# IML-DKFZ/values

Measured on AMD Instinct MI355X. Metric: uncertainty-volumes/sec (64^3, T=10 MC-dropout), higher is better.
Workload: dtype f32; 1 GPU; C2: 64^3 1-channel volumes, UNet3D(initial_filter_size=8, 2 classes), T=10 MC-dropout passes + fused softmax/entropy/MI/variance/argmax reduction; dropout=hash bit generator, new seed every step, weights=torch default init, seed 123

## Files before the change

### values_amd/csrc/conv3d_deep.hip

```cpp
#include "s16_common.h"
#include "conv3d_internal.h"

struct DeepArgs {
  vx_conv3d_args a;
  const float* w;
  int tx, ty, tz, ts;
  int ltx, lty, ltz;
  int tiles_x, tiles_y, tiles_z;
  int npos;
  int nchunks, ncg;
  int npairs;
  unsigned m_cg, m_tx, m_ty, m_tz;
  int stat_epc;
  unsigned long long* stamps;
  int abl;
};

#define DP_STAMP VX_STAMP
#define DP_WAIT_LOADS VX_STAMP_WAIT_LOADS
#define DP_ABL VX_DIAG(ka.abl)

constexpr int DEEP_PREC_B = DEEP_NPOS * 16;
constexpr int DEEP_IMG_B = 2 * DEEP_PREC_B;

template <int R, int EPI, int PRE>
__global__ __launch_bounds__(768) void conv3d_deep_kernel(DeepArgs ka) {
  constexpr int NW = 8, NPW = 4, NTH = (NW + NPW) * 64, NST = NPW * 64;
  constexpr int NT = 2, NSTEP = 7;
  constexpr int IN_IT = R == 4 ? 9 : 7;
  constexpr int W_IT = DEEP_W_B / 16 / NST;
  constexpr bool STATS = EPI == 0;

  extern __shared__ __attribute__((aligned(16))) unsigned char smem_raw[];
  unsigned char* s_img = smem_raw;
  unsigned char* s_w = smem_raw + 2 * DEEP_IMG_B;
  float* s_red = reinterpret_cast<float*>(s_w + 2 * DEEP_W_B);
  float* s_bias = s_red + 2 * NW * 32 * 2;

  const vx_conv3d_args& a = ka.a;
  auto kernarg = [&]() {
    typedef const DeepArgs __attribute__((address_space(4))) * kp_t;
    kp_t p = (kp_t)__builtin_amdgcn_kernarg_segment_ptr();
    asm volatile("" : "+s"(p));
    return p;
  };
  const int tid = threadIdx.x, lane = tid & 63;
  const int wave = __builtin_amdgcn_readfirstlane(tid >> 6);
  const int m = lane & 15, g = lane >> 4;
  const int TX = ka.tx, TY = ka.ty, TZ = ka.tz;
  const int HX = TX + 2, HY = TY + 2, HZ = TZ + 2;
  const int NCH = ka.nchunks;

  for (int i = tid; i < a.Cout; i += NTH) s_bias[i] = a.bias[i];

  int vb = blockIdx.x;
  const int G = (int)gridDim.x;
  if ((G & 7) == 0) vb = (blockIdx.x & 7) * (G >> 3) + (blockIdx.x >> 3);
  const int npair_wg = vb < ka.npairs ? (ka.npairs - vb + G - 1) / G : 0;

  struct Cur { int ci, c; };
  auto advance = [&](Cur& x) { if (++x.c == NCH) { x.c = 0; ++x.ci; } };
  auto pair_of = [&](int ci, int& n0, int& tzi, int& tyi, int& txi, int& cg) {
    unsigned t = (unsigned)(vb + ci * G), q;
    q = ka.ncg == 1 ? t : __umulhi(t, ka.m_cg); cg = (int)(t - q * (unsigned)ka.ncg); t = q;
    q = ka.tiles_x == 1 ? t : __umulhi(t, ka.m_tx); txi = (int)(t - q * (unsigned)ka.tiles_x); t = q;
    q = ka.tiles_y == 1 ? t : __umulhi(t, ka.m_ty); tyi = (int)(t - q * (unsigned)ka.tiles_y); t = q;
    q = ka.tiles_z == 1 ? t : __umulhi(t, ka.m_tz); tzi = (int)(t - q * (unsigned)ka.tiles_z);
    n0 = (int)q * ka.ts;
  };

  float rmax = 0.f;
#ifdef VX_CONV_STAMPS
  unsigned long long st_sum[8] = {0, 0, 0, 0, 0, 0, 0, 0}, st_last, st_iters = 0;
  asm volatile("s_memtime %0\n\ts_waitcnt lgkmcnt(0)" : "=s"(st_last)::"memory");
#endif

  if (wave >= NW) {
    if constexpr (PRE != 0 || R == 2) __builtin_amdgcn_s_setprio(2);
    const int t = tid - NW * 64;
    const int q = t & 1;
    const int xb = a.in_xblk;
    const int Csrc = xb ? a.Cin / 2 : a.Cin;
    const int voxf = xb ? 2 * Csrc : a.in_pitch;
    const int rowf = a.W * voxf;
    const int biasf = (a.H + 1) * rowf + 4 * voxf;
    const size_t in_sample = (size_t)a.D * a.H * rowf;
    const int cper = xb ? Csrc / 8 : 0;
    const int lastx = (ka.tiles_x - 1) * TX, lasty = (ka.tiles_y - 1) * TY, lastz = (ka.tiles_z - 1) * TZ;
    unsigned voff[IN_IT];
    int ldst[IN_IT];
    unsigned ibad_always = 0, ibad_xlo = 0, ibad_xhi = 0, ibad_ylo = 0, ibad_yhi = 0, ibad_zlo = 0, ibad_zhi = 0;
    unsigned ibad_sge[3] = {0, 0, 0};
#pragma unroll
    for (int it = 0; it < IN_IT; ++it) {
      const int idx = t + it * NST;
      int vox = idx >> 1;
      if (vox >= ka.npos) { ibad_always |= 1u << it; vox = 0; }
      const int hx = vox % HX, r1 = vox / HX;
      const int hy = r1 % HY, r2 = r1 / HY;
      const int hz = r2 % HZ, smp = r2 / HZ;
      const int dxr = hx - 1, dyr = hy - 1, dzr = hz - 1;
      int xf;
      if (xb) {
        const int blk = dxr >= 0 ? dxr / xb : -((-dxr + xb - 1) / xb);
        const int rem = dxr - blk * xb;
        xf = (blk * 2) * xb * Csrc + rem * Csrc + 4 * q;
      } else {
        xf = dxr * a.in_pitch + 4 * q;
      }
      voff[it] = (unsigned)(((size_t)smp * in_sample + (size_t)((dzr * a.H + dyr) * rowf + xf + biasf)) * 4);
      ldst[it] = vox * 16 + q * 8;
      if (dxr < 0) ibad_xlo |= 1u << it;
      if (dxr >= a.W - lastx) ibad_xhi |= 1u << it;
      if (dyr < 0) ibad_ylo |= 1u << it;
      if (dyr >= a.H - lasty) ibad_yhi |= 1u << it;
      if (dzr < 0) ibad_zlo |= 1u << it;
      if (dzr >= a.D - lastz) ibad_zhi |= 1u << it;
#pragma unroll
      for (int k = 0; k < 3; ++k)
        if (smp > k) ibad_sge[k] |= 1u << it;
    }
    const uint32_t seed_in = PRE == 1 ? vx_seed_of(a, a.in_drop_seed) : 0u;

    f32x4 ibuf[IN_IT];
    f32x4 p_mean = {0.f, 0.f, 0.f, 0.f}, p_rstd = {1.f, 1.f, 1.f, 1.f};
    unsigned p_bad = 0xFFFFFFFFu, p_e0 = 0;
    vx_dkey p_key = {0u, 0u};
    unsigned cs_bad = 0xFFFFFFFFu, cs_soff = 0;
    int cs_n = 0;
    __amdgpu_buffer_rsrc_t cs_srd = __builtin_amdgcn_make_buffer_rsrc((void*)a.in, 0, 0, 0x00020000);
    auto pair_state = [&](int ci) {
      const bool have = ci < npair_wg;
      int n0 = 0, tzi = 0, tyi = 0, txi = 0, cg = 0;
      if (have) pair_of(ci, n0, tzi, tyi, txi, cg);
      unsigned bad = ibad_always;
      if (txi == 0) bad |= ibad_xlo;
      if (txi == ka.tiles_x - 1) bad |= ibad_xhi;
      if (tyi == 0) bad |= ibad_ylo;
      if (tyi == ka.tiles_y - 1) bad |= ibad_yhi;
      if (tzi == 0) bad |= ibad_zlo;
      if (tzi == ka.tiles_z - 1) bad |= ibad_zhi;
      const int nv = a.N - n0;
      if (nv < ka.ts) bad |= ibad_sge[nv >= 1 ? nv - 1 : 0];
      if (!have) bad = 0xFFFFFFFFu;
      cs_bad = bad;
      cs_soff = (unsigned)((((tzi * TZ) * a.H + tyi * TY) * rowf + txi * TX * voxf) * 4);
// ... 201 lines not shown
        for (int nt = 0; nt < NT; ++nt)
#pragma unroll
          for (int j = 0; j < 4; ++j) { ssum[nt][j] = 0.f; ssq[nt][j] = 0.f; }
      }
      int m_ = m;
      asm volatile("" : "+v"(m_));
#pragma unroll
      for (int r = 0; r < R; ++r) {
        int cx_, ly, lz, smp;
        vox_of((wave * R + r) * 16 + m_, cx_, ly, lz, smp);
        const int ovox = (lz * a.H + ly) * a.W + cx_;
        unsigned ovoff_r = ((unsigned)smp * (unsigned)out_sample + (unsigned)ovox * (unsigned)out_voxf + (unsigned)kp->a.out_coff + 4u * g) * 4u;
        if constexpr (R == 2) {
          if (n0 + smp >= a.N) ovoff_r = VX_OOB;
        }
        uint32_t hword = 0;
        if (EPI == 1) {
          const vx_dkey key = vx_drop_key(seed_out, kp->a.drop_layer, (uint32_t)(n0 + smp));
          hword = vx_drop_word(key, (vox0 + (unsigned)ovox) * (unsigned)ka.ncg + (unsigned)cg) >> (4 * g);
        }
#pragma unroll
        for (int nt = 0; nt < NT; ++nt) {
          f32x4 v;
#pragma unroll
          for (int j = 0; j < 4; ++j) v[j] = fmaf(accx[r][nt][j], 1.0f / 2048.f, acc[r][nt][j]);
          if (STATS) {
#pragma unroll
            for (int j = 0; j < 4; ++j) { ssum[nt][j] += v[j]; ssq[nt][j] = fmaf(v[j], v[j], ssq[nt][j]); }
          }
          if (f_lrelu) {
#pragma unroll
            for (int j = 0; j < 4; ++j) v[j] = fmaxf(v[j], 0.01f * v[j]);
          } else if (f_relu) {
#pragma unroll
            for (int j = 0; j < 4; ++j) v[j] = fmaxf(v[j], 0.f);
          }
          if (EPI == 1) {
            const uint32_t bits = hword >> (16 * nt);
#pragma unroll
            for (int j = 0; j < 4; ++j) v[j] *= __uint_as_float((bits << (30 - j)) & 0x40000000u);
          }
          if (!STATS) rmax = vx_max3abs(vx_max3abs(rmax, v[0], v[1]), v[2], v[3]);
          u32x4 sv = __builtin_bit_cast(u32x4, v);
          if (EPI == 1 || EPI == 3) {
            if (a.out_split) {
              typedef unsigned u32x2 __attribute__((ext_vector_type(2)));
              f16x4 hi, lo;
              vx_split4_s(v, hi, lo);
              const u32x2 h2 = __builtin_bit_cast(u32x2, hi), l2 = __builtin_bit_cast(u32x2, lo);
              sv = (u32x4){h2[0], h2[1], l2[0], l2[1]};
            }
          }
          __builtin_amdgcn_raw_buffer_store_b128(sv, osrd, (int)ovoff_r, (int)(osoff + (unsigned)(nt * 64)), 0);
          __builtin_amdgcn_sched_barrier(0);
          asm volatile("s_nop 3" ::: "memory");
          __builtin_amdgcn_sched_barrier(0);
        }
      }
      if (STATS) {
#pragma unroll
        for (int nt = 0; nt < NT; ++nt)
#pragma unroll
          for (int j = 0; j < 4; ++j) {
            float s = ssum[nt][j], qq = ssq[nt][j];
#pragma unroll
            for (int rot = 8; rot >= 1; rot >>= 1) { s += vx_row_ror(s, rot); qq += vx_row_ror(qq, rot); }
            if (m == 0) {
              red[(wave * 32 + nt * 16 + g * 4 + j) * 2 + 0] = s;
              red[(wave * 32 + nt * 16 + g * 4 + j) * 2 + 1] = qq;
            }
          }
      }
    };

    auto flush_tile = [&](int ci) {
      const float* red = s_red + (ci & 1) * (NW * 32 * 2);
      int n0, tzi, tyi, txi, cg;
      pair_of(ci, n0, tzi, tyi, txi, cg);
      const auto kp = kernarg();
      const int epc = kp->stat_epc;
      const int tps = ka.tiles_x * ka.tiles_y * ka.tiles_z;
      const int tile = (tzi * ka.tiles_y + tyi) * ka.tiles_x + txi;
      float* dst = kp->a.stats_partial + (((size_t)n0 * tps + tile) * epc * a.Cout + cg * 32) * 2;
      if (tid < 32) {
        float s = 0.f, qq = 0.f;
#pragma unroll
        for (int w = 0; w < NW; ++w) {
          s += red[(w * 32 + tid) * 2 + 0];
          qq += red[(w * 32 + tid) * 2 + 1];
        }
        dst[tid * 2 + 0] = s;
        dst[tid * 2 + 1] = qq;
      }
      for (int e = 1; e < epc; ++e)
        if (tid < 64) dst[(size_t)e * a.Cout * 2 + tid] = 0.f;
    };

    const bool late = wave >= NW / 2;
    Cur cx = {0, 0};
    int j = 0;
    int prev_ci = -1;
    int fl_ci = -1, fl_at = 0;
    while (cx.ci < npair_wg) {
      __syncthreads();
      DP_STAMP(0);
      if (STATS && fl_ci >= 0 && j >= fl_at && !late) { flush_tile(fl_ci); fl_ci = -1; }
      if (late && prev_ci >= 0) {
        if (!(DP_ABL & 2)) epilogue(prev_ci);
        prev_ci = -1;
      }
      DP_STAMP(2);
      if (cx.c == 0) {
        int n0, tzi, tyi, txi, cg;
        pair_of(cx.ci, n0, tzi, tyi, txi, cg);
        const f32x4 zero = {0.f, 0.f, 0.f, 0.f};
#pragma unroll
        for (int nt = 0; nt < NT; ++nt) {
          const f32x4 b4 = *reinterpret_cast<const f32x4*>(s_bias + cg * 32 + nt * 16 + 4 * g);
#pragma unroll
          for (int r = 0; r < R; ++r) { acc[r][nt] = b4; accx[r][nt] = zero; }
        }
      }
      if (!(DP_ABL & 1)) multiply(j & 1);
      DP_STAMP(1);
      if (cx.c == NCH - 1) {
        if (late) prev_ci = cx.ci;
        else if (!(DP_ABL & 2)) epilogue(cx.ci);
        if (STATS) { fl_ci = cx.ci; fl_at = j + 2; }
      }
      DP_STAMP(2);
#ifdef VX_CONV_STAMPS
      ++st_iters;
#endif
      advance(cx);
      ++j;
    }
    if (late && prev_ci >= 0) epilogue(prev_ci);
    if (STATS) {
      __syncthreads();
      if (fl_ci >= 0 && !late) flush_tile(fl_ci);
    }
  }
  if (!STATS && a.range_flag) {
    float mx = rmax;
#pragma unroll
    for (int off = 32; off >= 1; off >>= 1) mx = fmaxf(mx, __shfl_xor(mx, off, 64));
    if (lane == 0 && !(mx < 32768.f)) atomicMax(a.range_flag, __float_as_uint(mx));
  }
#ifdef VX_CONV_STAMPS
  if (ka.stamps && lane == 0) {
    unsigned long long* d = ka.stamps + ((size_t)blockIdx.x * 16 + wave) * 8;
    for (int i = 0; i < 6; ++i) d[i] = st_sum[i];
    d[6] = st_iters;
  }
#endif
}

__global__ void pack_conv3d_deep_kernel(const float* __restrict__ w, _Float16* __restrict__ out, int Cin, int64_t total) {
  const int nch = Cin / 8;
  for (int64_t i = (int64_t)blockIdx.x * blockDim.x + threadIdx.x; i < total; i += (int64_t)gridDim.x * blockDim.x) {
    const int j = (int)(i & 7), lane = (int)((i >> 3) & 63), hl = (int)((i >> 9) & 1), nt = (int)((i >> 10) & 1);
    const int64_t sb = i >> 11;
    const int step = (int)(sb % 7);
    const int64_t blk = sb / 7;
    const int chunk = (int)(blk % nch), cg = (int)(blk / nch);
    const int row = cg * 32 + nt * 16 + (lane & 15), tap = 4 * step + (lane >> 4);
    const float v = tap > 26 ? 0.f : w[((size_t)row * Cin + 8 * chunk + j) * 27 + tap];
    const float c = fminf(fmaxf(v, -65504.f), 65504.f);
    const _Float16 h = (_Float16)c;
    out[i] = hl == 0 ? h : (_Float16)((v - (float)h) * 2048.f);
  }
}

int vx_pack_conv3d_deep(const float* w_torch, float* w_packed, int Cin, int Cout, hipStream_t s) {
  const int64_t total = conv3d_deep_packed_floats(Cin, Cout) * 2;
  if (total <= 0) return VX_OK;
  int blocks = (int)((total + 255) / 256);
  if (blocks > 4096) blocks = 4096;
  hipLaunchKernelGGL(pack_conv3d_deep_kernel, dim3(blocks), dim3(256), 0, s, w_torch, reinterpret_cast<_Float16*>(w_packed), Cin, total);
  VX_CHECK_LAUNCH("vx_pack_conv3d_k3(deep)");
  return VX_OK;
}

template <int R, int EPI, int PRE>
static int launch_deep(const DeepArgs& ka, const Conv3dRoute& r, hipStream_t s) {
  constexpr size_t lds = 2 * (size_t)DEEP_IMG_B + 2 * (size_t)DEEP_W_B + 2 * 8 * 32 * 2 * 4 + DEEP_MAXC * 4;
  static_assert(lds <= 160 * 1024, "LDS budget");
  auto kern = conv3d_deep_kernel<R, EPI, PRE>;
  static bool attr = false;
  if (!attr) {
    hipError_t e = hipFuncSetAttribute(reinterpret_cast<const void*>(kern), hipFuncAttributeMaxDynamicSharedMemorySize, (int)lds);
    if (e != hipSuccess) VX_FAIL((int)e, "vx_conv3d_k3(deep): hipFuncSetAttribute(%zu B LDS): %s", lds, hipGetErrorString(e));
    attr = true;
  }
  int gx = vx_cu_count();
  if (gx > ka.npairs) gx = ka.npairs;
  static const char* kname = vx_conv3d_kname(r);
  vx_note_kernel(kname);
  hipLaunchKernelGGL(kern, dim3((unsigned)gx), dim3(768), lds, s, ka);
  VX_CHECK_LAUNCH("vx_conv3d_k3(deep)");
  return VX_OK;
}

int vx_conv3d_deep_launch(const Conv3dRoute& r, const vx_conv3d_args& a, const float* w_block, hipStream_t s) {
  DeepArgs ka;
  ka.a = a;
  ka.w = w_block;
  ka.tx = r.tx; ka.ty = r.ty; ka.tz = r.tz; ka.ts = r.ts;
  ka.ltx = __builtin_ctz((unsigned)r.tx); ka.lty = __builtin_ctz((unsigned)r.ty); ka.ltz = __builtin_ctz((unsigned)r.tz);
  ka.tiles_x = r.tiles_x; ka.tiles_y = r.tiles_y; ka.tiles_z = r.tiles_z;
  ka.npos = r.npos;
  ka.nchunks = r.nchunks;
  ka.ncg = r.ncg;
  ka.npairs = r.nitems;
  ka.m_cg = r.m_cg; ka.m_tx = r.mx; ka.m_ty = r.my; ka.m_tz = r.mz;
  ka.stat_epc = r.stat_epc;
  vx_conv_diag(VX_DIAG_XP_ABL, &ka.stamps, &ka.abl);
  switch (conv3d_key_of(r.p, r.np)) {
#define DEEP_CASE(...) case conv3d_key(__VA_ARGS__): return launch_deep<__VA_ARGS__>(ka, r, s);
    DEEP_INSTANCES(DEEP_CASE)
#undef DEEP_CASE
  }
  VX_FAIL(VX_E_SHAPE, "vx_conv3d_k3(deep): no such instance");
}
```

### values_amd/csrc/conv3d_route.h

```cpp
#pragma once
#include <stdint.h>
#include <stdio.h>

#include "../../include/values_amd.h"
#include "host_checks.h"

constexpr int DEEP_NPOS = 1080;
constexpr int DEEP_NPOS_R2 = 896;
constexpr int DEEP_W_B = 7 * 2 * 2 * 1024;
constexpr int DEEP_MAXC = 512;
constexpr int DEEP_MAXDIM = 32;
constexpr int S16_HEAD_MAXC = 4;

enum Conv3dKernel { CONV3D_MFMA = 0, CONV3D_C8, CONV3D_S16, CONV3D_XP8W, CONV3D_ZC16, CONV3D_DEEP, CONV3D_NKERNELS };

#define MFMA_TILES(X, CB, NT, XP) X(CB, NT, 16, 4, 4, 8, XP) X(CB, NT, 8, 8, 4, 8, XP) X(CB, NT, 4, 4, 4, 4, XP)
#define MFMA_INSTANCES(X) MFMA_TILES(X, 8, 1, 1) MFMA_TILES(X, 16, 1, 0) MFMA_TILES(X, 16, 2, 0) MFMA_TILES(X, 8, 1, 0) MFMA_TILES(X, 8, 2, 0)
#define C8_INSTANCES(X) X(1, 32, 4, 4) X(2, 32, 4, 4) X(1, 16, 8, 4) X(2, 16, 8, 4) X(1, 8, 4, 4) X(2, 8, 4, 4)
#define S16_SMALL(X, CB, NT, XP)                                                                                       \
  X(CB, NT, 16, 4, 4, 8, XP, 0, 0) X(CB, NT, 16, 4, 4, 8, XP, 0, 1) X(CB, NT, 16, 4, 4, 8, XP, 0, 3)                     \
  X(CB, NT, 8, 8, 4, 8, XP, 0, 0) X(CB, NT, 8, 8, 4, 8, XP, 0, 1) X(CB, NT, 8, 8, 4, 8, XP, 0, 3) X(CB, NT, 4, 4, 4, 4, XP, 0, 3)
#define S16_LARGE(X, CB, XP) X(CB, 1, 16, 8, 4, 8, XP, 0, 0) X(CB, 1, 16, 8, 4, 8, XP, 0, 1) X(CB, 1, 16, 8, 4, 8, XP, 0, 3)
#define S16_DB_PLAIN(X, CB, NT) X(CB, NT, 16, 4, 4, 8, 0, 2, 0) X(CB, NT, 16, 4, 4, 8, 0, 2, 1) X(CB, NT, 16, 4, 4, 8, 0, 2, 3)
#define S16_DB_XP(X)                                                                                                   \
  X(8, 1, 16, 8, 4, 8, 1, 2, 0) X(8, 1, 16, 8, 4, 8, 1, 2, 1) X(8, 1, 16, 8, 4, 8, 1, 2, 2) X(8, 1, 16, 8, 4, 8, 1, 2, 3) \
  X(8, 1, 16, 8, 4, 8, 1, 3, 1) X(8, 1, 16, 8, 4, 8, 1, 3, 3)
#define S16_INSTANCES_PART0(X) S16_SMALL(X, 16, 1, 0) S16_LARGE(X, 16, 0) S16_DB_PLAIN(X, 16, 1)
#define S16_INSTANCES_PART1(X)                                                                                         \
  S16_SMALL(X, 8, 1, 1) S16_LARGE(X, 8, 1) S16_DB_XP(X) S16_SMALL(X, 8, 1, 0) S16_LARGE(X, 8, 0) S16_DB_PLAIN(X, 8, 1) \
  S16_SMALL(X, 8, 2, 0) S16_DB_PLAIN(X, 8, 2)
#define S16_INSTANCES_PART2(X) S16_SMALL(X, 16, 2, 0) S16_DB_PLAIN(X, 16, 2)
#define S16_INSTANCES(X) S16_INSTANCES_PART0(X) S16_INSTANCES_PART1(X) S16_INSTANCES_PART2(X)
#define XP8W_INSTANCES(X)                                                                                              \
  X(1, 4, 0, 0, 4, 0) X(1, 4, 1, 0, 4, 0) X(1, 4, 2, 0, 4, 0) X(1, 0, 2, 0, 4, 0) X(1, 0, 0, 0, 4, 0) X(1, 0, 1, 0, 4, 0)  \
  X(1, 1, 0, 0, 4, 0) X(1, 2, 0, 0, 4, 0) X(1, 3, 0, 0, 4, 0) X(1, 3, 1, 0, 4, 0) X(1, 5, 0, 0, 4, 0)                      \
  X(2, 1, 0, 0, 8, 0) X(2, 1, 1, 0, 8, 0) X(2, 3, 0, 0, 8, 0) X(2, 3, 1, 0, 8, 0)                                          \
  X(2, 1, 0, 1, 8, 0) X(2, 1, 1, 1, 8, 0) X(2, 3, 0, 1, 8, 0) X(2, 3, 1, 1, 8, 0)                                          \
  X(2, 1, 0, 2, 8, 0) X(2, 1, 1, 2, 8, 0) X(2, 3, 0, 2, 8, 0) X(2, 3, 1, 2, 8, 0)                                          \
  X(1, 2, 0, 0, 4, 1) X(1, 2, 0, 0, 4, 3) X(1, 4, 2, 0, 4, 2) X(2, 1, 1, 2, 8, 2)
#define ZC16_INSTANCES(X)                                                                                              \
  X(16, 0, 0, 0, 0) X(16, 0, 1, 0, 0) X(16, 4, 0, 0, 0) X(16, 4, 1, 0, 0) X(16, 1, 0, 0, 0) X(16, 1, 1, 0, 0)              \
  X(16, 3, 0, 0, 0) X(16, 3, 1, 0, 0) X(16, 1, 4, 0, 0) X(16, 3, 4, 0, 0) X(16, 5, 0, 0, 0) X(16, 6, 0, 0, 0)              \
  X(8, 0, 0, 0, 0) X(8, 0, 3, 0, 0) X(8, 3, 0, 0, 0) X(8, 1, 0, 0, 0)                                                      \
  X(16, 1, 0, 1, 0) X(16, 3, 0, 1, 0) X(16, 1, 0, 0, 1) X(16, 3, 0, 0, 1)                                                  \
  X(16, 1, 0, 1, 1) X(16, 3, 0, 1, 1) X(16, 5, 0, 1, 1) X(16, 6, 0, 1, 1)
#define DEEP_INSTANCES(X) X(4, 0, 0) X(4, 0, 1) X(4, 1, 0) X(4, 3, 0) X(2, 0, 0) X(2, 0, 1) X(2, 1, 0) X(2, 3, 0)

constexpr uint64_t conv3d_key(int a, int b = 0, int c = 0, int d = 0, int e = 0, int f = 0, int g = 0, int h = 0, int i = 0) {
  return ((((((((uint64_t)a * 64 + b) * 64 + c) * 64 + d) * 64 + e) * 64 + f) * 64 + g) * 64 + h) * 64 + i;
}
static inline uint64_t conv3d_key_of(const int* p, int np) {
  int q[9] = {0, 0, 0, 0, 0, 0, 0, 0, 0};
  for (int i = 0; i < np; ++i) q[i] = p[i];
  return conv3d_key(q[0], q[1], q[2], q[3], q[4], q[5], q[6], q[7], q[8]);
}
#define CONV3D_EXISTS_CASE(...) case conv3d_key(__VA_ARGS__):
static inline bool conv3d_instance_exists(int kernel, const int* p, int np) {
  const uint64_t key = conv3d_key_of(p, np);
  switch (kernel) {
    case CONV3D_MFMA: switch (key) { MFMA_INSTANCES(CONV3D_EXISTS_CASE) return true; default: return false; }
    case CONV3D_C8:   switch (key) { C8_INSTANCES(CONV3D_EXISTS_CASE) return true; default: return false; }
    case CONV3D_S16:  switch (key) { S16_INSTANCES(CONV3D_EXISTS_CASE) return true; default: return false; }
    case CONV3D_XP8W: switch (key) { XP8W_INSTANCES(CONV3D_EXISTS_CASE) return true; default: return false; }
    case CONV3D_ZC16: switch (key) { ZC16_INSTANCES(CONV3D_EXISTS_CASE) return true; default: return false; }
    case CONV3D_DEEP: switch (key) { DEEP_INSTANCES(CONV3D_EXISTS_CASE) return true; default: return false; }
  }
  return false;
}

struct Conv3dRoute {
  int kernel;
  int np, p[9];
  int64_t w_off;
  int tiles_x, tiles_y, tiles_z;
  unsigned mx, my, mz;
  int nchunks;
  int ty8;
  int kz;
  int nitems;
  unsigned mcps;
  int rep; unsigned mrep;
  int stat_epc;
  int tx, ty, tz, ts, npos, ncg;
  unsigned m_cg;
  char err[400];
};

static inline bool conv3d_pow2(int64_t v) { return (v & (v - 1)) == 0; }
constexpr int64_t CONV3D_2GIB = 1ll << 31;

struct S16Cfg { int CB, NT, XP; };
static inline S16Cfg s16_config(int Cin, int Cout) {
  S16Cfg c;
  c.NT = (Cout % 32 == 0) ? 2 : 1;
  c.XP = Cout == 8 ? 1 : 0;
  c.CB = c.XP ? 8 : ((Cin % 16 == 0) ? 16 : 8);
  return c;
}
static inline bool conv3d_c8_applies(int Cin, int Cout) { return Cout == 8 && (Cin == 8 || Cin == 16); }
struct ConvCfg { int CB, NT, XP, C8, S16; };
static inline ConvCfg conv_config(int Cin, int Cout, const vx_config& cfg) {
  const S16Cfg s = s16_config(Cin, Cout);
  ConvCfg c;
  c.CB = s.CB; c.NT = s.NT; c.XP = s.XP;
  c.S16 = (cfg.conv_fp32 == 0 || (cfg.conv_fp32 == 2 && Cout != 8)) ? 1 : 0;
  c.C8 = (!c.S16 && conv3d_c8_applies(Cin, Cout)) ? 1 : 0;
  return c;
}
static inline bool conv3d_channels_ok(int Cin, int Cout) { return Cin > 0 && Cout > 0 && Cin % 8 == 0 && Cout % 8 == 0; }
static inline int64_t conv_rows_padded(int Cout, int NT) { return (((int64_t)Cout + 16 * NT - 1) / (16 * NT)) * (16 * NT); }
static inline bool conv3d_s16_head_fusable(int Cin, int Cout) { return s16_config(Cin, Cout).XP != 0; }
static inline bool conv3d_s16_prologue_ok(int Cin, int Cout) { return s16_config(Cin, Cout).XP == 0; }

static inline bool conv3d_zc16_packs(int Cin, int Cout) { return Cout == 16 && (Cin == 8 || Cin == 16); }
static inline bool conv3d_deep_packs(int Cin, int Cout) { return Cout % 32 == 0 && Cin % 8 == 0 && Cin >= 16 && Cout <= DEEP_MAXC; }

static inline bool conv3d_xp8_applies(int D, int H, int W, int Cin, int Cout, const vx_config& cfg) {
  if (cfg.conv_fp32 != 0 || cfg.s16_no_xp8) return false;
  return Cout == 8 && (Cin == 8 || Cin == 16) && W % 32 == 0 && H % 8 == 0 && D % 4 == 0 && W >= 32 && H >= 8 && D >= 8;
}
static inline bool conv3d_zc16_applies(int D, int H, int W, int Cin, int Cout, const vx_config& cfg) {
  if (cfg.conv_fp32 != 0 || cfg.s16_no_zc16) return false;
  return conv3d_zc16_packs(Cin, Cout) && W % 32 == 0 && H % 8 == 0 && D % 2 == 0 && W >= 32 && H >= 8 && D >= 4;
}
struct DeepGeo { int tx, ty, tz, ts, tiles_x, tiles_y, tiles_z, npos; };
static inline bool deep_geo(int D, int H, int W, int R, DeepGeo* o) {
  const int vox = 128 * R;
  const int tx = W < 16 ? W : 16;
  if (tx < 4 || !conv3d_pow2(tx) || W % tx) return false;
  int ty = H < 8 ? H : 8;
  while (tx * ty > vox) ty >>= 1;
  if (ty < 1 || H % ty) return false;
  int tz = vox / (tx * ty);
  if (tz > D) tz = D;
  if (tz < 1 || D % tz) return false;
  const int ts = vox / (tx * ty * tz);
  if (ts * tx * ty * tz != vox) return false;
  if (!conv3d_pow2(ty) || !conv3d_pow2(tz)) return false;
  if (ts > 1 && (tx != W || ty != H || tz != D || ts > 4 || R != 2)) return false;
  const int npos = ts * (tx + 2) * (ty + 2) * (tz + 2);
  if (npos > (R == 4 ? DEEP_NPOS : DEEP_NPOS_R2)) return false;
  o->tx = tx; o->ty = ty; o->tz = tz; o->ts = ts;
  o->tiles_x = W / tx; o->tiles_y = H / ty; o->tiles_z = D / tz; o->npos = npos;
  return true;
}
static inline int deep_pick(int D, int H, int W, DeepGeo* o) {
  if (deep_geo(D, H, W, 4, o)) return 4;
  return deep_geo(D, H, W, 2, o) ? 2 : 0;
}
static inline bool conv3d_deep_applies(int D, int H, int W, int Cin, int Cout, const vx_config& cfg) {
  if (cfg.conv_fp32 != 0 || cfg.s16_no_deep) return false;
  if (!conv3d_deep_packs(Cin, Cout)) return false;
  if (W > DEEP_MAXDIM || H > DEEP_MAXDIM || D > DEEP_MAXDIM) return false;
  DeepGeo g;
  return deep_pick(D, H, W, &g) != 0;
}

struct TileCfg { int TX, TY, TZ, TXV; };
static inline TileCfg tile_config(int W, int XP) {
  if (XP) {
    if (W >= 32) return {16, 4, 4, 32};
    if (W >= 16) return {8, 8, 4, 16};
    return {4, 4, 4, 8};
  }
  if (W >= 16) return {16, 4, 4, 16};
  if (W >= 8) return {8, 8, 4, 8};
  return {4, 4, 4, 4};
}
static inline void vx_conv3d_s16_tile(int H, int W, int Cout, int* txv, int* ty, int* tz) {
  const int xp = s16_config(8, Cout).XP;
  const int wcols = xp ? W / 2 : W;
  const int tx = wcols >= 16 ? 16 : (wcols >= 8 ? 8 : 4);
  const bool nt2 = !xp && Cout % 32 == 0;
  const bool ty8 = tx == 16 && H >= 32 && !nt2;
  *txv = xp ? 2 * tx : tx;
  *ty = (tx == 8 || ty8) ? 8 : 4;
  *tz = 4;
}
static inline int conv3d_tiles_along(int n, int t) { return (int)(((int64_t)n + t - 1) / t); }
static inline int conv3d_tile_count(int D, int H, int W, int txv, int ty, int tz) {
  return (int)((unsigned)conv3d_tiles_along(W, txv) * (unsigned)conv3d_tiles_along(H, ty) * (unsigned)conv3d_tiles_along(D, tz));
}
static inline int conv3d_tiles_for(int D, int H, int W, int Cout, const vx_config& cfg) {
  if (conv_config(8, Cout, cfg).S16) {
    int txv, ty, tz;
    vx_conv3d_s16_tile(H, W, Cout, &txv, &ty, &tz);
    return conv3d_tile_count(D, H, W, txv, ty, tz);
  }
  const TileCfg t = tile_config(W, Cout == 8);
  return conv3d_tile_count(D, H, W, t.TXV, t.TY, t.TZ);
}
static inline int conv3d_tiles_max(int D, int H, int W) {
  int best = 0;
  for (int xp = 0; xp < 2; ++xp) {
    const TileCfg t = tile_config(W, xp);
    const int n = conv3d_tile_count(D, H, W, t.TXV, t.TY, t.TZ);
    if (n > best) best = n;
  }
  const int couts[3] = {8, 16, 32};
  for (int i = 0; i < 3; ++i) {
    int txv, ty, tz;
    vx_conv3d_s16_tile(H, W, couts[i], &txv, &ty, &tz);
    const int n = conv3d_tile_count(D, H, W, txv, ty, tz);
    if (n > best) best = n;
  }
  return best;
}

static inline int64_t conv3d_s16_packed_floats(int Cin, int Cout) {
  const S16Cfg c = s16_config(Cin, Cout);
  const int TPS = 32 / c.CB, NSTEP = c.XP ? 9 : (27 + TPS - 1) / TPS;
  const int64_t halves = (int64_t)(conv_rows_padded(Cout, c.NT) / 16) * (Cin / c.CB) * NSTEP * 2 * (c.XP ? 32 : 64) * 8;
  return halves / 2;
}
static inline int64_t conv3d_zc16_packed_floats(int Cin, int Cout) {
  return conv3d_zc16_packs(Cin, Cout) ? (int64_t)(Cin == 16 ? 14 : 9) * 2 * 64 * 8 / 2 : 0;
}
static inline int64_t conv3d_deep_packed_floats(int Cin, int Cout) {
  return conv3d_deep_packs(Cin, Cout) ? (int64_t)(Cout / 32) * (Cin / 8) * (DEEP_W_B / 4) : 0;
}
static inline int conv3d_family(int Cin, int Cout, const vx_config& cfg) {
  if (!conv3d_channels_ok(Cin, Cout)) return 0;
  const ConvCfg c = conv_config(Cin, Cout, cfg);
  if (c.S16) {
    if (c.XP) return 2;
    if (conv3d_deep_packs(Cin, Cout)) return 7;
    return conv3d_zc16_packs(Cin, Cout) ? 6 : 1;
  }
  if (c.C8) return 5;
  return c.XP ? 4 : 3;
}
static inline int64_t conv3d_packed_floats(int Cin, int Cout, const vx_config& cfg) {
// ... 107 lines not shown
                     a.act, a.drop_mode, a.stats_partial ? 1 : 0);
  if (a.pool_out) VX_REFUSE(r, VX_E_SHAPE, "vx_conv3d_k3(xp8w): no pooled output for this epilogue");
  return ROUTE_DECLINED;
}

static inline int route_zc16(const vx_conv3d_args& a, int stat_tiles, Conv3dRoute* r) {
  if (a.in_xblk || a.head_out || a.in_split || a.in_f16 || a.out_f16 || (a.in_repeat > 1)) return ROUTE_DECLINED;
  if ((a.in_planar || a.out_planar) && (a.drop_mode == VX_DROP_MASK || !a.out || a.in_pitch != a.Cin || a.Cout != 16))
    VX_REFUSE(r, VX_E_SHAPE, "vx_conv3d_k3(zc16): the planar pre-split hand-over needs hash or no dropout and dense 16-channel tensors");
  if (a.up_in && (a.Cin != 16 || a.in_mean || a.stats_partial || a.up_pitch < 32 || a.up_pitch % 4 || (a.up_fused && (!a.acc_in || a.out_xblk || a.out_split))))
    VX_REFUSE(r, VX_E_SHAPE, "vx_conv3d_k3(zc16): the fused up-convolution (32 coarse channels -> the conv's 16 input channels) goes with an "
               "activation epilogue, no prologue, up_pitch >= 32 (got %d), up_w packed by vx_pack_convT_zc16; composed weights "
               "(up_fused: vx_pack_conv3d_upfused_zc16) only together with partial sums (acc_in) and a dense float or planar output", a.up_pitch);
  if (a.drop_mode == VX_DROP_MASK || !a.out) return ROUTE_DECLINED;
  route_columns(r, a, 2, stat_tiles);
  const int cps = r->tiles_x * r->tiles_y;
  if ((int64_t)a.N * cps >= (1ll << 31)) VX_REFUSE(r, VX_E_SHAPE, "vx_conv3d_k3(zc16): too many columns");
  if (a.in_pitch != a.Cin) return ROUTE_DECLINED;
  if (a.stats_partial && (stat_tiles % cps || a.act != VX_ACT_NONE || (a.drop_mode != VX_DROP_NONE && !a.pool_out)))
    VX_REFUSE(r, VX_E_SHAPE, "vx_conv3d_k3(zc16): statistics go with a plain epilogue");
  if (a.pool_out && (!a.stats_partial || a.Cin != 16)) VX_REFUSE(r, VX_E_SHAPE, "vx_conv3d_k3(zc16): the pooled output goes with statistics, 16 -> 16");
  int pre = 0;
  if (a.in_pool_flags) pre = 3;
  else if (a.in_mean) pre = 1;
  if ((pre == 1 && a.Cin != 16) || (pre == 3 && a.Cin != 8)) return ROUTE_DECLINED;
  if (a.in_planar) {
    if (a.Cin != 16 || pre != 0 || a.up_in || a.acc_in || a.stats_partial || !vx_aligned16(a.in) ||
        (vx_wide)a.D * a.H * a.W * 64 >= CONV3D_2GIB)
      VX_REFUSE(r, VX_E_SHAPE, "vx_conv3d_k3(zc16): a planar pre-split input (in_planar) goes with 16 -> 16, an activation epilogue, no "
                 "prologue / up-convolution / partial sums, a 16-byte aligned tensor, one sample below 2 GiB");
    pre = 4;
  }
  if (a.out_planar && (a.stats_partial || a.out_pitch != 16 || a.out_coff != 0 || a.out_xblk || a.out_split || a.out == a.acc_in ||
                       (vx_wide)a.D * a.H * a.W * 64 >= CONV3D_2GIB))
    VX_REFUSE(r, VX_E_SHAPE, "vx_conv3d_k3(zc16): a planar pre-split output (out_planar) goes with an activation epilogue into a dense "
               "16-channel tensor that is not the partial sums' (another layout), one sample below 2 GiB");
  int epi;
  if (a.stats_partial) epi = a.pool_out ? 4 : 0;
  else if (a.drop_mode == VX_DROP_HASH) { if (a.act != VX_ACT_LRELU) return ROUTE_DECLINED; epi = 1; }
  else epi = 3;
  if (a.out_split && a.stats_partial) VX_REFUSE(r, VX_E_SHAPE, "vx_conv3d_k3(zc16): out_split goes with the activation epilogues");
  if (a.out_planar) {
    if (a.Cin != 16 || pre != 0 || (epi != 1 && epi != 3) || ((a.acc_in != nullptr) != (a.up_in != nullptr)))
      VX_REFUSE(r, VX_E_SHAPE, "vx_conv3d_k3(zc16): out_planar goes with 16 -> 16, an activation epilogue, no prologue, and either partial "
                 "sums + the fused up-convolution together or neither");
    epi = epi == 1 ? 5 : 6;
  }
  if (a.acc_in && (a.Cin != 16 || pre != 0 || a.stats_partial || a.acc_pitch < 16 || a.acc_pitch % 4 || !vx_aligned16(a.acc_in) ||
                   (vx_wide)a.D * a.H * a.W * a.acc_pitch * 4 >= CONV3D_2GIB))
    VX_REFUSE(r, VX_E_SHAPE, "vx_conv3d_k3(zc16): partial sums (acc_in) go with 16 -> 16, no prologue, an activation epilogue, a "
               "16-byte aligned tensor of pitch >= 16 (pitch %d), one sample below 2 GiB", a.acc_pitch);
  route_instance(r, CONV3D_ZC16, 5, a.Cin, epi, pre, a.acc_in ? 1 : 0, a.up_in ? 1 : 0);
  if (conv3d_instance_exists(CONV3D_ZC16, r->p, 5)) return VX_OK;
  if (a.up_in && !a.acc_in) VX_REFUSE(r, VX_E_SHAPE, "vx_conv3d_k3(zc16): no fused up-convolution for this epilogue");
  return ROUTE_DECLINED;
}

static inline int route_deep(const vx_conv3d_args& a, int stat_tiles, Conv3dRoute* r) {
  if (a.head_out || a.in_split || a.in_f16 || a.out_f16 || (a.in_repeat > 1) || a.out_xblk || a.up_in || a.pool_out ||
      a.in_pool_flags || a.acc_in)
    return ROUTE_DECLINED;
  if (a.drop_mode == VX_DROP_MASK || !a.out) return ROUTE_DECLINED;
  DeepGeo g;
  const int R = deep_pick(a.D, a.H, a.W, &g);
  if (!R) return ROUTE_DECLINED;
  if (a.in_xblk) {
    const int csrc = a.Cin / 2;
    if (a.in_mean || csrc % 8 || a.W % a.in_xblk) return ROUTE_DECLINED;
  } else if (a.in_pitch % 4) {
    return ROUTE_DECLINED;
  }
  if (a.in_mean && (a.in_pitch != a.Cin || g.ts != 1)) return ROUTE_DECLINED;
  if (a.stats_partial && g.ts != 1) return ROUTE_DECLINED;
  r->tx = g.tx; r->ty = g.ty; r->tz = g.tz; r->ts = g.ts; r->npos = g.npos;
  r->tiles_x = g.tiles_x; r->tiles_y = g.tiles_y; r->tiles_z = g.tiles_z;
  r->nchunks = a.Cin / 8;
  r->ncg = a.Cout / 32;
  const int tps = g.tiles_x * g.tiles_y * g.tiles_z;
  const int64_t npairs = (((int64_t)a.N + g.ts - 1) / g.ts) * tps * r->ncg;
  if (npairs >= (1ll << 31)) VX_REFUSE(r, VX_E_SHAPE, "vx_conv3d_k3(deep): too many tiles");
  r->nitems = (int)npairs;
  r->m_cg = vx_magic_raw(r->ncg); r->mx = vx_magic_raw(g.tiles_x); r->my = vx_magic_raw(g.tiles_y); r->mz = vx_magic_raw(g.tiles_z);
  r->stat_epc = 0;
  if (a.stats_partial) {
    if (stat_tiles % tps) return ROUTE_DECLINED;
    if (a.act != VX_ACT_NONE || a.drop_mode != VX_DROP_NONE) VX_REFUSE(r, VX_E_SHAPE, "vx_conv3d_k3(deep): statistics go with a plain epilogue");
    r->stat_epc = stat_tiles / tps;
  }
  if ((vx_wide)g.ts * a.D * a.H * a.W * a.out_pitch * 4 >= CONV3D_2GIB)
    VX_REFUSE(r, VX_E_SHAPE, "vx_conv3d_k3(deep): one tile's samples must stay below 2 GiB");
  int epi;
  if (a.stats_partial) epi = 0;
  else if (a.drop_mode == VX_DROP_HASH) { if (a.act != VX_ACT_LRELU) return ROUTE_DECLINED; epi = 1; }
  else epi = 3;
  if (a.out_split && a.stats_partial) VX_REFUSE(r, VX_E_SHAPE, "vx_conv3d_k3(deep): out_split goes with the activation epilogues");
  route_instance(r, CONV3D_DEEP, 3, R, epi, a.in_mean ? 1 : 0);
  return conv3d_instance_exists(CONV3D_DEEP, r->p, 3) ? VX_OK : ROUTE_DECLINED;
}

static inline int route_s16(const vx_conv3d_args& a, const vx_config& cfg, Conv3dRoute* r) {
  const S16Cfg c = s16_config(a.Cin, a.Cout);
  int txv, ty, tz;
  vx_conv3d_s16_tile(a.H, a.W, a.Cout, &txv, &ty, &tz);
  const int tx = c.XP ? txv / 2 : txv;
  route_tiles(r, a, txv, ty, tz);
  r->nchunks = a.Cin / c.CB;
  r->ty8 = (tx == 16 && ty == 8) ? 1 : 0;
  const bool generic = cfg.s16_generic != 0;
  int epi = 3;
  if (generic) epi = 3;
  else if (a.act == VX_ACT_NONE && a.drop_mode == VX_DROP_NONE && !a.head_out && a.out) epi = 0;
  else if (a.act == VX_ACT_LRELU && a.drop_mode == VX_DROP_HASH && !a.head_out && a.out) epi = 1;
  else if (a.act == VX_ACT_LRELU && a.drop_mode == VX_DROP_HASH && a.head_out && c.XP) epi = 2;
  int db = 0;
  if (!generic && tx == 16 && c.XP && r->ty8 && r->nchunks <= 2) db = r->nchunks == 1 ? 2 : 3;
  if (!generic && tx == 16 && !c.XP && !r->ty8 && r->nchunks == 1) db = 2;
  if (epi == 2 && db != 2) epi = 3;
  if (db == 3 && epi == 0) epi = 3;
  if (tx == 4) epi = 3;
  route_instance(r, CONV3D_S16, 9, c.CB, c.NT, tx, ty, tz, tx == 4 ? 4 : 8, c.XP, db, epi);
  if (!conv3d_instance_exists(CONV3D_S16, r->p, 9)) VX_REFUSE(r, VX_E_SHAPE, "vx_conv3d_k3(s16): no instance for this tile");
  return VX_OK;
}

static inline int conv3d_route(const vx_conv3d_args& a, const vx_config& cfg, Conv3dRoute* r) {
  r->err[0] = 0;
  r->w_off = 0;
  if (!a.in || !a.w_packed || !a.bias || (!a.out && !a.head_out)) VX_REFUSE(r, VX_E_NULL, "vx_conv3d_k3: null tensor pointer");
  const ConvCfg c = conv_config(a.Cin, a.Cout, cfg);
  if (a.head_out) {
    if (!a.head_w || !a.head_b) VX_REFUSE(r, VX_E_NULL, "vx_conv3d_k3: fused head without weights");
    if (a.head_C < 1 || a.head_C > 8) VX_REFUSE(r, VX_E_SHAPE, "vx_conv3d_k3: fused head takes 1..8 classes, got %d", a.head_C);
    if (c.S16 && a.head_C > S16_HEAD_MAXC)
      VX_REFUSE(r, VX_E_SHAPE, "vx_conv3d_k3: the split-fp16 kernel fuses heads of up to 4 classes, got %d", a.head_C);
    if (!conv3d_head_fusable(a.Cin, a.Cout, cfg))
      VX_REFUSE(r, VX_E_SHAPE, "vx_conv3d_k3: no fused head for Cin=%d Cout=%d (see vx_conv3d_k3_head_fusable)", a.Cin, a.Cout);
    if (a.stats_partial) VX_REFUSE(r, VX_E_SHAPE, "vx_conv3d_k3: fused head on a layer with InstanceNorm statistics");
  }
  if (!conv3d_channels_ok(a.Cin, a.Cout))
    VX_REFUSE(r, VX_E_SHAPE, "vx_conv3d_k3: Cin=%d Cout=%d must be positive multiples of 8", a.Cin, a.Cout);
  if (a.N <= 0 || a.D <= 0 || a.H <= 0 || a.W <= 0) VX_REFUSE(r, VX_E_SHAPE, "vx_conv3d_k3: empty tensor");
  if (a.w_family != conv3d_family(a.Cin, a.Cout, cfg))
    VX_REFUSE(r, VX_E_DTYPE, "vx_conv3d_k3: weights packed for kernel family %d, the library is configured for family %d "
               "(vx_conv3d_k3_family(%d, %d)): re-pack them", a.w_family, conv3d_family(a.Cin, a.Cout, cfg), a.Cin, a.Cout);
  if (a.out_xblk && ((a.out_xblk != 1 && a.out_xblk != 2 && a.out_xblk != 4) || a.W % a.out_xblk || (a.out_half != 0 && a.out_half != 1)))
    VX_REFUSE(r, VX_E_SHAPE, "vx_conv3d_k3: bad concat output (xblk=%d, half=%d, W=%d)", a.out_xblk, a.out_half, a.W);
  if ((a.in_mean == nullptr) != (a.in_rstd == nullptr)) VX_REFUSE(r, VX_E_NULL, "vx_conv3d_k3: in_mean / in_rstd must come together");
  if (a.products != 0 && a.products != 1 && a.products != 3)
    VX_REFUSE(r, VX_E_SHAPE, "vx_conv3d_k3: products = %d (0 / 3: the default split scheme, 1: one fp16 product)", a.products);
  const bool xp8 = c.S16 && conv3d_xp8_applies(a.D, a.H, a.W, a.Cin, a.Cout, cfg) && a.drop_mode != VX_DROP_MASK;
  if (a.products == 1 && !(xp8 && a.in_drop_mode != VX_DROP_MASK))
    VX_REFUSE(r, VX_E_SHAPE, "vx_conv3d_k3: products = 1 is taken by the full-resolution z-column kernel only (got %dx%dx%d, %d -> %d)",
               a.D, a.H, a.W, a.Cin, a.Cout);
  if ((a.in_planar || a.out_planar) && !conv3d_zc16_16to16(a.D, a.H, a.W, a.Cin, a.Cout, cfg))
    VX_REFUSE(r, VX_E_SHAPE, "vx_conv3d_k3: the planar pre-split hand-over (in_planar / out_planar) is taken where vx_conv3d_k3_planar_ok "
               "(got %dx%dx%d, %d -> %d)", a.D, a.H, a.W, a.Cin, a.Cout);
  if (a.up_in) {
    if (!a.up_w || !a.up_b) VX_REFUSE(r, VX_E_NULL, "vx_conv3d_k3: fused up-convolution without weights");
    if (!conv3d_upfuse_ok(a.D, a.H, a.W, a.Cin, a.Cout, cfg) || a.drop_mode == VX_DROP_MASK || a.stats_partial || a.head_out)
      VX_REFUSE(r, VX_E_SHAPE, "vx_conv3d_k3: no fused up-convolution for this layer (see vx_conv3d_k3_upfuse_ok; hash or no "
                 "dropout, no statistics, no head): %dx%dx%d, %d -> %d", a.D, a.H, a.W, a.Cin, a.Cout);
    if (a.up_pitch < 16 || a.up_pitch % 4 || !vx_aligned16(a.up_in) || !vx_aligned16(a.up_b))
      VX_REFUSE(r, VX_E_ALIGN, "vx_conv3d_k3: up_in pitch %d (>= 16, multiple of 4 floats) / alignment", a.up_pitch);
    if ((vx_wide)(a.D / 2 + 2) * (a.H / 2) * (a.W / 2) * a.up_pitch * 4 >= CONV3D_2GIB)
      VX_REFUSE(r, VX_E_SHAPE, "vx_conv3d_k3: one coarse sample must stay below 2 GiB");
    if (a.up_fused && !vx_aligned16(a.up_fused)) VX_REFUSE(r, VX_E_ALIGN, "vx_conv3d_k3: up_fused alignment");
  } else if (a.up_fused) {
    VX_REFUSE(r, VX_E_SHAPE, "vx_conv3d_k3: up_fused (composed up-convolution weights) without up_in");
  }
  if (a.pool_out) {
// ... 84 lines not shown
```

Before: 3930 volumes/s.

## Split tail work-items across multiple workgroups in deep conv kernel

Result: faster. 3973 volumes/s (median of 6 runs) (+1.1%).

```diff
diff --git a/values_amd/csrc/conv3d_deep.hip b/values_amd/csrc/conv3d_deep.hip
--- a/values_amd/csrc/conv3d_deep.hip
+++ b/values_amd/csrc/conv3d_deep.hip
@@ -9,9 +9,10 @@
   int tiles_x, tiles_y, tiles_z;
   int npos;
   int nchunks, ncg;
-  int npairs;
   unsigned m_cg, m_tx, m_ty, m_tz;
   int stat_epc;
+  int stat_parts;
+  int nfull, tail0, tail_wgs, ltail;
   unsigned long long* stamps;
   int abl;
 };
@@ -56,12 +57,14 @@
   int vb = blockIdx.x;
   const int G = (int)gridDim.x;
   if ((G & 7) == 0) vb = (blockIdx.x & 7) * (G >> 3) + (blockIdx.x >> 3);
-  const int npair_wg = vb < ka.npairs ? (ka.npairs - vb + G - 1) / G : 0;
+  const int nfull = ka.nfull;
+  const int npair_wg = nfull + (vb < ka.tail_wgs ? 1 : 0);
 
   struct Cur { int ci, c; };
   auto advance = [&](Cur& x) { if (++x.c == NCH) { x.c = 0; ++x.ci; } };
   auto pair_of = [&](int ci, int& n0, int& tzi, int& tyi, int& txi, int& cg) {
     unsigned t = (unsigned)(vb + ci * G), q;
+    if (ci >= nfull) { const auto kp = kernarg(); t = (unsigned)(kp->tail0 + (vb >> kp->ltail)); }
     q = ka.ncg == 1 ? t : __umulhi(t, ka.m_cg); cg = (int)(t - q * (unsigned)ka.ncg); t = q;
     q = ka.tiles_x == 1 ? t : __umulhi(t, ka.m_tx); txi = (int)(t - q * (unsigned)ka.tiles_x); t = q;
     q = ka.tiles_y == 1 ? t : __umulhi(t, ka.m_ty); tyi = (int)(t - q * (unsigned)ka.tiles_y); t = q;
@@ -429,21 +432,29 @@
       const int tps = ka.tiles_x * ka.tiles_y * ka.tiles_z;
       const int tile = (tzi * ka.tiles_y + tyi) * ka.tiles_x + txi;
       float* dst = kp->a.stats_partial + (((size_t)n0 * tps + tile) * epc * a.Cout + cg * 32) * 2;
-      if (tid < 32) {
+      const int parts = kp->stat_parts, wpp = NW / parts;
+      const int ltail = kp->ltail;
+      const bool shared = ci >= nfull && ltail > 0;
+      const int p = tid >> 5, ch = tid & 31;
+      if (p < parts && (!shared || (p * wpp) >> (3 - ltail) == (vb & ((1 << ltail) - 1)))) {
         float s = 0.f, qq = 0.f;
 #pragma unroll
-        for (int w = 0; w < NW; ++w) {
-          s += red[(w * 32 + tid) * 2 + 0];
-          qq += red[(w * 32 + tid) * 2 + 1];
-        }
-        dst[tid * 2 + 0] = s;
-        dst[tid * 2 + 1] = qq;
-      }
-      for (int e = 1; e < epc; ++e)
-        if (tid < 64) dst[(size_t)e * a.Cout * 2 + tid] = 0.f;
+        for (int i = 0; i < NW; ++i) {
+          const int w = (p * wpp + i) & (NW - 1);
+          const float rs = red[(w * 32 + ch) * 2 + 0], rq = red[(w * 32 + ch) * 2 + 1];
+          s = i < wpp ? s + rs : s;
+          qq = i < wpp ? qq + rq : qq;
+        }
+        dst[(size_t)p * a.Cout * 2 + ch * 2 + 0] = s;
+        dst[(size_t)p * a.Cout * 2 + ch * 2 + 1] = qq;
+      }
+      if (!shared || (vb & ((1 << ltail) - 1)) == 0)
+        for (int e = parts; e < epc; ++e)
+          if (tid < 64) dst[(size_t)e * a.Cout * 2 + tid] = 0.f;
     };
 
     const bool late = wave >= NW / 2;
+    const bool tail_mine = (wave >> (3 - ka.ltail)) == (vb & ((1 << ka.ltail) - 1));
     Cur cx = {0, 0};
     int j = 0;
     int prev_ci = -1;
@@ -457,7 +468,8 @@
         prev_ci = -1;
       }
       DP_STAMP(2);
-      if (cx.c == 0) {
+      const bool mine = cx.ci < nfull || tail_mine;
+      if (cx.c == 0 && mine) {
         int n0, tzi, tyi, txi, cg;
         pair_of(cx.ci, n0, tzi, tyi, txi, cg);
         const f32x4 zero = {0.f, 0.f, 0.f, 0.f};
@@ -468,11 +480,13 @@
           for (int r = 0; r < R; ++r) { acc[r][nt] = b4; accx[r][nt] = zero; }
         }
       }
-      if (!(DP_ABL & 1)) multiply(j & 1);
+      if (mine && !(DP_ABL & 1)) multiply(j & 1);
       DP_STAMP(1);
       if (cx.c == NCH - 1) {
-        if (late) prev_ci = cx.ci;
-        else if (!(DP_ABL & 2)) epilogue(cx.ci);
+        if (mine) {
+          if (late) prev_ci = cx.ci;
+          else if (!(DP_ABL & 2)) epilogue(cx.ci);
+        }
         if (STATS) { fl_ci = cx.ci; fl_at = j + 2; }
       }
       DP_STAMP(2);
@@ -530,7 +544,7 @@
 }
 
 template <int R, int EPI, int PRE>
-static int launch_deep(const DeepArgs& ka, const Conv3dRoute& r, hipStream_t s) {
+static int launch_deep(const DeepArgs& ka, const Conv3dRoute& r, int grid, hipStream_t s) {
   constexpr size_t lds = 2 * (size_t)DEEP_IMG_B + 2 * (size_t)DEEP_W_B + 2 * 8 * 32 * 2 * 4 + DEEP_MAXC * 4;
   static_assert(lds <= 160 * 1024, "LDS budget");
   auto kern = conv3d_deep_kernel<R, EPI, PRE>;
@@ -540,11 +554,9 @@
     if (e != hipSuccess) VX_FAIL((int)e, "vx_conv3d_k3(deep): hipFuncSetAttribute(%zu B LDS): %s", lds, hipGetErrorString(e));
     attr = true;
   }
-  int gx = vx_cu_count();
-  if (gx > ka.npairs) gx = ka.npairs;
   static const char* kname = vx_conv3d_kname(r);
   vx_note_kernel(kname);
-  hipLaunchKernelGGL(kern, dim3((unsigned)gx), dim3(768), lds, s, ka);
+  hipLaunchKernelGGL(kern, dim3((unsigned)grid), dim3(768), lds, s, ka);
   VX_CHECK_LAUNCH("vx_conv3d_k3(deep)");
   return VX_OK;
 }
@@ -559,12 +571,14 @@
   ka.npos = r.npos;
   ka.nchunks = r.nchunks;
   ka.ncg = r.ncg;
-  ka.npairs = r.nitems;
   ka.m_cg = r.m_cg; ka.m_tx = r.mx; ka.m_ty = r.my; ka.m_tz = r.mz;
   ka.stat_epc = r.stat_epc;
+  ka.stat_parts = r.stat_parts;
+  const DeepTail t = deep_tail(r.nitems, vx_cu_count(), r.tail_cap);
+  ka.nfull = t.full; ka.tail0 = t.tail0; ka.tail_wgs = t.rest * t.split; ka.ltail = __builtin_ctz((unsigned)t.split);
   vx_conv_diag(VX_DIAG_XP_ABL, &ka.stamps, &ka.abl);
   switch (conv3d_key_of(r.p, r.np)) {
-#define DEEP_CASE(...) case conv3d_key(__VA_ARGS__): return launch_deep<__VA_ARGS__>(ka, r, s);
+#define DEEP_CASE(...) case conv3d_key(__VA_ARGS__): return launch_deep<__VA_ARGS__>(ka, r, t.grid, s);
     DEEP_INSTANCES(DEEP_CASE)
 #undef DEEP_CASE
   }
diff --git a/values_amd/csrc/conv3d_route.h b/values_amd/csrc/conv3d_route.h
--- a/values_amd/csrc/conv3d_route.h
+++ b/values_amd/csrc/conv3d_route.h
@@ -81,6 +81,7 @@
   unsigned mcps;
   int rep; unsigned mrep;
   int stat_epc;
+  int stat_parts, tail_cap;
   int tx, ty, tz, ts, npos, ncg;
   unsigned m_cg;
   char err[400];
@@ -148,6 +149,20 @@
   if (deep_geo(D, H, W, 4, o)) return 4;
   return deep_geo(D, H, W, 2, o) ? 2 : 0;
 }
+struct DeepTail { int full, rest, split, tail0, grid; };
+static inline DeepTail deep_tail(int P, int G, int cap) {
+  DeepTail t;
+  if (G < 1) G = 1;
+  t.full = P / G;
+  t.tail0 = t.full * G;
+  t.rest = P - t.tail0;
+  t.split = 1;
+  for (int s = 4; s >= 2; s >>= 1)
+    if (t.split == 1 && s <= cap && t.rest > 0 && (int64_t)t.rest * s <= G) t.split = s;
+  t.grid = t.full > 0 ? G : t.rest * t.split;
+  return t;
+}
+static inline int deep_stat_parts(int stat_epc) { return stat_epc >= 4 ? 4 : (stat_epc >= 2 ? 2 : 1); }
 static inline bool conv3d_deep_applies(int D, int H, int W, int Cin, int Cout, const vx_config& cfg) {
   if (cfg.conv_fp32 != 0 || cfg.s16_no_deep) return false;
   if (!conv3d_deep_packs(Cin, Cout)) return false;
@@ -421,10 +436,13 @@
   r->nitems = (int)npairs;
   r->m_cg = vx_magic_raw(r->ncg); r->mx = vx_magic_raw(g.tiles_x); r->my = vx_magic_raw(g.tiles_y); r->mz = vx_magic_raw(g.tiles_z);
   r->stat_epc = 0;
+  r->stat_parts = 1;
+  r->tail_cap = 4;
   if (a.stats_partial) {
     if (stat_tiles % tps) return ROUTE_DECLINED;
     if (a.act != VX_ACT_NONE || a.drop_mode != VX_DROP_NONE) VX_REFUSE(r, VX_E_SHAPE, "vx_conv3d_k3(deep): statistics go with a plain epilogue");
     r->stat_epc = stat_tiles / tps;
+    r->tail_cap = r->stat_parts = deep_stat_parts(r->stat_epc);
   }
   if ((vx_wide)g.ts * a.D * a.H * a.W * a.out_pitch * 4 >= CONV3D_2GIB)
     VX_REFUSE(r, VX_E_SHAPE, "vx_conv3d_k3(deep): one tile's samples must stay below 2 GiB");
```
